# NVIDIA/DeepLearningExamples

Measured on AMD Instinct MI355X. Metric: training samples/sec, higher is better.
Workload: dtype bf16; 1 GPU; ResNet-50 v1.5 (PyTorch/Classification/ConvNets) synthetic ImageNet 224x224, label smoothing 0.1, SGD momentum 0.875 (BASELINE.json configs[1]); batch_per_gpu=256, global_batch=256, layout=NHWC, hip_graph=False, parallelism=single GPU

## Files before the change

### deeplearningexamples_amd/_cabi.py

```python
import ctypes
import os

import torch

_HERE = os.path.dirname(os.path.abspath(__file__))
LIB_PATH = os.environ.get("DLE_LIB_PATH") or os.path.join(_HERE, "lib", "libdle_mi355x.so")

F32, F16, BF16 = 0, 1, 2
ACT_NONE, ACT_RELU, ACT_GELU, ACT_RELU_BWD, ACT_ADD, ACT_GELU_BWD, ACT_TANH, ACT_TANH_BWD = 0, 1, 2, 3, 4, 5, 6, 7
ACT_ADD_MASKED, ACT_MUL, ACT_GELU_DAUX = 8, 9, 10

_DT = {torch.float32: F32, torch.float16: F16, torch.bfloat16: BF16}

c_void_p, c_int, c_i64, c_float = ctypes.c_void_p, ctypes.c_int, ctypes.c_int64, ctypes.c_float
c_u64 = ctypes.c_uint64

_SIGS = {
    "dle_last_error": (ctypes.c_char_p, []),
    "dle_abi_version": (c_int, []),
    "dle_device_check": (c_int, [c_int, ctypes.c_char_p, c_int]),
    "dle_dot_interact_out_width": (c_int, [c_int, c_int]),
    "dle_dot_interact_fwd": (c_int, [c_void_p, c_void_p, c_int, c_int, c_int, c_int, c_int, c_void_p]),
    "dle_dot_interact_bwd": (c_int, [c_void_p, c_void_p, c_void_p, c_void_p, c_int, c_int, c_int, c_int,
                                     c_int, c_void_p]),
# ... 17 lines not shown
    "dle_emb_sgd_workspace_bytes": (c_i64, [c_void_p, c_int, c_int, c_i64]),
    "dle_emb_onehot_try": (c_int, [c_void_p, c_void_p, c_void_p, c_void_p, c_float, c_void_p, c_void_p, c_void_p, c_void_p,
                                   c_void_p, c_int, c_i64, c_int, c_int, c_i64, c_int, c_void_p, c_i64, c_void_p]),
    "dle_emb_onehot_partials": (c_int, [c_void_p, c_void_p, c_void_p, c_void_p, c_void_p, c_void_p, c_int, c_i64, c_int, c_int,
                                        c_i64, c_int, c_void_p, c_i64, c_void_p, c_void_p]),
    "dle_emb_adam_workspace_bytes": (c_i64, [c_void_p, c_int, c_int, c_i64]),
    "dle_emb_adam_dedup_ws": (c_int, [c_void_p] * 9 + [c_float, c_void_p, c_void_p, c_void_p, c_float, c_float, c_float, c_i64,
                                      c_int, c_int, c_i64, c_int, c_void_p, c_i64, c_void_p]),
    "dle_cast_rows": (c_int, [c_void_p, c_void_p, c_i64, c_int, c_int, c_i64, c_i64, c_int, c_int, c_void_p]),
    "dle_bce_logits": (c_int, [c_void_p, c_void_p, c_void_p, c_void_p, c_void_p, c_i64, c_i64, c_int, c_void_p]),
    "dle_conv1x1_bnbwd_dgrad": (c_int, [c_void_p] * 16 + [c_i64, c_int, c_int, c_int, c_int, c_void_p]),
    "dle_conv1x1_bnbwd_groups": (c_int, [c_int]),
    "dle_conv1x1_bnbwd_dgrad_wgrad": (c_int, [c_void_p] * 15 + [c_i64, c_void_p, c_void_p, c_void_p, c_i64, c_int, c_int, c_int, c_int,
                                              c_void_p]),
    "dle_conv1x1_bnbwd_wgrad_workspace": (c_i64, [c_int, c_int]),
    "dle_gemm_expand_masked_bnred": (c_int, [c_void_p] * 10 + [c_i64, c_int, c_int, c_int, c_i64, c_i64, c_i64, c_int, c_int, c_void_p]),
    "dle_bn_bwd_finish": (c_int, [c_void_p, c_int, c_int, c_void_p, c_void_p, c_int, c_void_p]),
    "dle_gemm_colsum": (c_int, [c_void_p, c_void_p, c_void_p, c_void_p, c_void_p, c_int, c_int, c_int, c_i64, c_i64, c_i64, c_int,
                                c_int, c_int, c_void_p, c_i64, c_void_p]),
    "dle_head_bce_workspace_bytes": (c_i64, [c_i64, c_int]),
    "dle_head_bce_fwd_bwd": (c_int, [c_void_p, c_void_p, c_void_p, c_void_p, c_void_p, c_void_p, c_void_p, c_void_p, c_void_p,
                                     c_void_p, c_void_p, c_void_p, c_i64, c_i64, c_int, c_i64, c_i64, c_int, c_void_p]),
    "dle_amp_update_scale": (c_int, [c_void_p, c_void_p, c_void_p, c_void_p, c_float, c_float, c_int, c_int,
                                     c_void_p]),
    "dle_check_nonfinite": (c_int, [c_void_p, c_void_p, c_i64, c_int, c_void_p]),
    "dle_axpby_f32": (c_int, [c_void_p, c_void_p, c_void_p, c_float, c_float, c_i64, c_void_p]),
    "dle_act_bwd": (c_int, [c_void_p, c_void_p, c_void_p, c_i64, c_int, c_int, c_void_p]),
    "dle_relu_bwd": (c_int, [c_void_p, c_void_p, c_void_p, c_i64, c_int, c_i64, c_i64, c_i64, c_int, c_void_p]),
    "dle_gemm": (c_int, [c_void_p, c_void_p, c_void_p, c_void_p, c_void_p, c_void_p, c_int, c_int, c_int,
                         c_i64, c_i64, c_i64, c_int, c_int, c_int, c_int, c_int, c_int, c_int, c_float,
# ... 339 lines not shown
```

### deeplearningexamples_amd/convnets/resnet.py

```python
from contextlib import nullcontext as _nullcontext
from typing import List

import os

import torch
from torch import nn

from .. import _cabi as C
from .. import functional as F

LAYERS, WIDTHS, EXPANSION = [3, 4, 6, 3], [64, 128, 256, 512], 4


def _conv(cin, cout, k, stride, device):
    m = nn.Conv2d(cin, cout, kernel_size=k, stride=stride, padding=(k - 1) // 2, bias=False, device=device)
    nn.init.kaiming_normal_(m.weight, mode="fan_in", nonlinearity="relu")
    m.weight.data = m.weight.data.contiguous(memory_format=torch.channels_last)
    return m


def _bn(c, device, zero_init=False):
    m = nn.BatchNorm2d(c, device=device)
    nn.init.constant_(m.weight, 0 if zero_init else 1)
    nn.init.constant_(m.bias, 0)
# ... 29 lines not shown

class ConvBN:

    def __init__(self, conv: nn.Conv2d, bn: nn.BatchNorm2d, name_conv: str, name_bn: str, relu: bool):
        self.conv, self.bn, self.name_conv, self.name_bn, self.relu = conv, bn, name_conv, name_bn, relu
        self.k = conv.kernel_size[0]
        self.stride, self.pad = conv.stride[0], conv.padding[0]
        self.cin, self.cout = conv.in_channels, conv.out_channels
        self.w16 = None
        self.gw = self.ggamma = self.gbeta = None
        self.saved = None
        self.w2 = self.gw_flat = None
        self.wgrad_stream = None
        self.fuse_bnbwd = os.environ.get("DLE_RN50_FUSE_BNBWD", "1") != "0"
        self.fuse_bnbwd_wgrad = os.environ.get("DLE_RN50_FUSE_BNBWD_WGRAD", "1") != "0"
        self.reduce_done = False
        self.keepalive = None

    def forward(self, x, residual=None, defer=False):
        t = None
        if isinstance(x, Deferred):
            d, r = x, None
            if self.k == 1 and self.stride == 1 and d.unit.relu and d.y is None:
                res, res_bn = d.residual_args()
                r = F.conv1x1_bnload_fwd(d.t, res, self.w16, d.mean, d.rstd, d.unit.bn.weight.data, d.unit.bn.bias.data,
                                         self.bn.running_mean, self.bn.running_var, eps=self.bn.eps, momentum=self.bn.momentum,
                                         res_bn=res_bn)
            if r is not None:
                t, x, bits, mean, rstd = r
                d._done(x, bits)
# ... 35 lines not shown
        fused = None
        wgrad_done = False
        if self.fuse_bnbwd and self.k == 1 and self.stride == 1 and need_dx and dx_addend is None:
            b2 = None
            if bnred is not None and bnred.saved is not None and bnred.relu:
                b2 = (bnred.saved[1], bnred.saved[2], bnred.saved[3], bnred.saved[4], bnred.ggamma, bnred.gbeta)
            if self.fuse_bnbwd_wgrad and pooled is None and self.gw is not None:
                r = F.bn_bwd_conv1x1_dgrad_wgrad(dy, t, mean, rstd, self.bn.weight.data, self.ggamma, self.gbeta,
                                                 self.w16.view(self.cout, c), x, self.gw, relu_mask=rmask,
                                                 reduce_done=reduce_done, bnred=b2)
                if r is not None:
                    fused, wgrad_done = (None, r[0], r[1]), True
            if fused is None:
                fused = F.bn_bwd_conv1x1_dgrad(dy, t, mean, rstd, self.bn.weight.data, self.ggamma, self.gbeta,
                                               self.w16.view(self.cout, c), relu_mask=rmask, reduce_done=reduce_done, bnred=b2)
        gt = None
        if pooled is not None:
            if self.relu and not reduce_done:
                gt = F.pool_bn_bwd(pooled[0], pooled[1], t, mean, rstd, self.bn.weight.data, self.ggamma, self.gbeta, rmask)
            if gt is None:
                dy = F.maxpool_bwd(pooled[0], pooled[1], t.shape[1:3])
        if gt is not None:
            pass
        elif fused is not None:
            gt = fused[0]
            if fused[2]:
                bnred.reduce_done = True
        else:
            gt, _ = F.bn_bwd(dy, None, t, mean, rstd, self.bn.weight.data, self.ggamma, self.gbeta, relu_mask=rmask,
                             reduce_done=reduce_done)
# ... 110 lines not shown
```

### deeplearningexamples_amd/csrc/conv_bnbwd.hip

```cpp
#include "gemm_tiles.h"

#define BB_PAD 8

struct BnbArgs {
  const unsigned short* DY;
  const unsigned short* T;
  const unsigned char* bits;
  const unsigned short* B;
  unsigned short* DT;
  unsigned short* C;
  const float* mean; const float* rstd; const float* gamma; const float* dgamma; const float* dbeta;
  float inv_m;
  int M, N, K;
  int row_tiles, groups;
  const unsigned short* X;
  float* wpartial;
  float* tile_part;
  const unsigned short* t2;
  const unsigned char* bits2;
  const float* mean2; const float* rstd2;
  float* partial;
};

template <int DT> struct BbMfma;
// ... 51 lines not shown
  float* mu2 = cf + 5 * K;
  constexpr int WG_BASE = TN * LDW * 2 + 5 * K * 4 + 2 * TN * 4, LD = K * 2, LX = TN * 2;
  constexpr int KSL = K / NW, KB = KSL / 32, CB = TN / 32, MS = TM / 16, XP = TM * LX / 16 / (NW * 64);
  static_assert(!WG || (WG_BASE % 256 == 0 && KS == 8 && NB == 4 && XP * NW * 64 * 16 == TM * LX), "LDS image of the weight-gradient tile");
  unsigned char* dtl = smem_raw + WG_BASE;
  unsigned char* xl = dtl + TM * LD;
  const int lane = threadIdx.x & 63, wave = threadIdx.x >> 6;
  const int fr = lane & 15, kg = lane >> 4;
  const int g = blockIdx.x;
  for (int c = threadIdx.x; c < K * (TN / 8); c += NW * 64) {
    const int k = c / (TN / 8), nc = c - k * (TN / 8);
    const ushort8_t v = *(const ushort8_t*)(p.B + (long long)k * p.N + nc * 8);
#pragma unroll
    for (int e = 0; e < 8; ++e) wl[bb_pos(nc * 8 + e) * LDW + k] = v[e];
  }
  for (int c = threadIdx.x; c < K; c += NW * 64) {
    const float rs = p.rstd[c];
    cf[c] = p.gamma[c] * rs;
    cf[K + c] = p.mean[c];
    cf[2 * K + c] = rs;
    cf[3 * K + c] = p.dbeta[c] * p.inv_m;
    cf[4 * K + c] = p.dgamma[c] * p.inv_m;
  }
  if (BRED) {
    for (int c = threadIdx.x; c < TN; c += NW * 64) { mu2[c] = p.mean2[c]; mu2[TN + c] = p.rstd2[c]; }
  }
  __syncthreads();
  const unsigned short* wrow = wl + fr * LDW + kg * 8;
  const int mrow = wave * 16 + fr;
  ushort8_t fg[KS], fx[KS];
  uint4_t mb0, mb1;
  ushort8_t t2c[BRED ? NP : 1];
  uint2_t m2c;
  float r1 = 0.f, r2 = 0.f;
  ushort8_t xr[WG ? XP : 1];
  float16_t wacc[WG ? KB : 1][WG ? CB : 1];
  if constexpr (WG) {
#pragma unroll
// ... 30 lines not shown
#pragma unroll
      for (int i = 0; i < XP; ++i) {
        const int c = threadIdx.x + i * NW * 64, xm = tmn * TM + (c >> 3);
        xr[i] = *(const ushort8_t*)(p.X + (long long)(xm < p.M ? xm : p.M - 1) * TN + (c & 7) * 8);
      }
    }
  };
  load_rows(g);
  for (int tm = g; tm < p.row_tiles; tm += p.groups) {
    const int m_cur = tm * TM + mrow;
    const bool live = m_cur < p.M;
    {
      const long long o = (long long)(live ? m_cur : 0) * K + kg * 8;
#pragma unroll
      for (int ks = 0; ks < KS; ++ks) {
        const int c0 = ks * 32 + kg * 8;
        float gf[8], xf[8], of[8];
        unpack8<DT>(fg[ks], gf);
        unpack8<DT>(fx[ks], xf);
        const unsigned mw = ks < 4 ? mb0[ks & 3] : mb1[ks & 3];
        const unsigned bits = MASK ? (mw >> (8 * kg)) & 0xffu : 0xffu;
#pragma unroll
        for (int k = 0; k < 8; ++k) {
          if (MASK) { if (!((bits >> k) & 1u)) gf[k] = 0.f; }
          const float xh = (xf[k] - cf[K + c0 + k]) * cf[2 * K + c0 + k];
          of[k] = cf[c0 + k] * (gf[k] - cf[3 * K + c0 + k] - xh * cf[4 * K + c0 + k]);
        }
        fg[ks] = pack8<DT>(of);
        if constexpr (!WG) { if (live) *(ushort8_t*)(p.DT + o + ks * 32) = fg[ks]; }
      }
    }
    if constexpr (WG) {
      lds_barrier();
      const ushort8_t zero8 = {0, 0, 0, 0, 0, 0, 0, 0};
#pragma unroll
      for (int ks = 0; ks < KS; ++ks)
        *(ushort8_t*)(dtl + mrow * LD + (((ks * 2 + (kg >> 1)) ^ (2 * (mrow & 3))) << 5) + (kg & 1) * 16) = live ? fg[ks] : zero8;
#pragma unroll
      for (int i = 0; i < XP; ++i) {
        const int c = threadIdx.x + i * NW * 64, r = c >> 3, ch = c & 7;
        *(ushort8_t*)(xl + r * LX + (((ch >> 1) ^ (2 * ((r >> 1) & 1))) << 5) + (ch & 1) * 16) = tm * TM + r < p.M ? xr[i] : zero8;
      }
      lds_barrier();
// ... 240 lines not shown
```

### deeplearningexamples_amd/csrc/gemm_expand.hip

```cpp
#include "gemm_tiles.h"

#define EX_TN 128
#define EX_PAD 8

struct ExpandArgs {
  const unsigned short* A;
  const unsigned short* B;
  unsigned short* C;
  const unsigned short* src;
  const unsigned char* bits;
  float* stats;
  int M, N, K;
  long long lda, ldb, ldc;
  int b_kc, row_tiles, groups, col_tiles;
  FastDiv dHW, dW;
  int up_HW, up_W, up_P, up_Q;
  long long ld_src;
  const unsigned short* t2;
  const unsigned char* bits2;
  const float* mean2;
  const float* rstd2;
};

template <int DT> struct ExMfma;
template <> struct ExMfma<DLE_F16> {
  static __device__ __forceinline__ float4_t run(ushort8_t a, ushort8_t b, float4_t c) {
    return __builtin_amdgcn_mfma_f32_16x16x32_f16(__builtin_bit_cast(half8_t, a), __builtin_bit_cast(half8_t, b), c, 0, 0, 0);
  }
};
template <> struct ExMfma<DLE_BF16> {
  static __device__ __forceinline__ float4_t run(ushort8_t a, ushort8_t b, float4_t c) {
    return __builtin_amdgcn_mfma_f32_16x16x32_bf16(__builtin_bit_cast(bf16x8_t, a), __builtin_bit_cast(bf16x8_t, b), c, 0, 0, 0);
  }
};

__device__ __forceinline__ int ex_pos(int nl) {
  const int j = nl >> 5, r = nl & 31;
  return 32 * j + 16 * ((r >> 2) & 1) + 4 * (r >> 3) + (r & 3);
}

template <int KS, int ACT, bool BRED = false>
struct ExStream {
  ushort8_t fa[KS];
  ushort8_t sv[ACT ? 4 : 1];
  ushort8_t tv[BRED ? 4 : 1];
  uint4_t mb;
  uint4_t mb2;
  long long o0;
  bool live;
  bool has;
  __device__ __forceinline__ void load_a(const ExpandArgs& p, int m, int kg) {
    const long long mr = m < p.M ? m : p.M - 1;
    const unsigned short* arow = p.A + mr * p.lda + kg * 8;
#pragma unroll
    for (int ks = 0; ks < KS; ++ks) fa[ks] = *(const ushort8_t*)(arow + ks * 32);
  }
  __device__ __forceinline__ void load_src(const ExpandArgs& p, int m, int n0, int kg) {
    live = m < p.M;
    const long long mr = live ? m : p.M - 1;
    o0 = mr * p.ldc + n0 + kg * 8;
    if (ACT == 3) {
      const int mi = (int)mr;
      const int n = fd_div(mi, p.dHW), rem = mi - n * p.up_HW;
      const int h = fd_div(rem, p.dW), w = rem - h * p.up_W;
      has = !((h | w) & 1);
      const long long cr = has ? ((long long)n * p.up_P + (h >> 1)) * p.up_Q + (w >> 1) : 0;
      const unsigned short* srow = p.src + cr * p.ld_src + n0 + kg * 8;
#pragma unroll
      for (int j = 0; j < 4; ++j) sv[j] = *(const ushort8_t*)(srow + 32 * j);
    } else if (ACT) {
// ... 22 lines not shown
    const float keep = h4 ? w16[8 + q] : w16[q], send = h4 ? w16[q] : w16[8 + q];
    w8[q] = keep + __shfl_xor(send, 4, 64);
  }
#pragma unroll
  for (int q = 0; q < 4; ++q) {
    const float keep = h2 ? w8[4 + q] : w8[q], send = h2 ? w8[q] : w8[4 + q];
    w4[q] = keep + __shfl_xor(send, 2, 64);
  }
#pragma unroll
  for (int q = 0; q < 2; ++q) {
    const float keep = h1 ? w4[2 + q] : w4[q], send = h1 ? w4[q] : w4[2 + q];
    acc[q] += keep + __shfl_xor(send, 1, 64);
  }
}

template <int DT, int KS, int ACT, bool STATS, int NW, bool BRED = false>
__global__ __launch_bounds__(NW * 64) __attribute__((amdgpu_waves_per_eu((STATS || BRED) ? 3 : 4)))
void gemm_expand_kernel(ExpandArgs p) {
  constexpr int K = KS * 32, LDW = K + EX_PAD, TM = NW * 16;
  extern __shared__ __attribute__((aligned(16))) unsigned char smem_raw[];
  unsigned short* wl = (unsigned short*)smem_raw;
  const int lane = threadIdx.x & 63, wave = threadIdx.x >> 6;
  const int fr = lane & 15, kg = lane >> 4;
  const int xcd = blockIdx.x & 7, slot = blockIdx.x >> 3;
  const int tn = slot % p.col_tiles, g = (slot / p.col_tiles) * 8 + xcd;
  const int n0 = tn * EX_TN;
  if (p.b_kc) {
    constexpr int CPR = K / 8;
    for (int c = threadIdx.x; c < EX_TN * CPR; c += NW * 64) {
      const int nl = c / CPR, kc = c - nl * CPR;
      const ushort8_t v = *(const ushort8_t*)(p.B + (long long)(n0 + nl) * p.ldb + kc * 8);
      *(ushort8_t*)(wl + ex_pos(nl) * LDW + kc * 8) = v;
    }
  } else {
    for (int c = threadIdx.x; c < K * (EX_TN / 8); c += NW * 64) {
      const int k = c >> 4, nc = c & 15;
      const ushort8_t v = *(const ushort8_t*)(p.B + (long long)k * p.ldb + n0 + nc * 8);
#pragma unroll
      for (int e = 0; e < 8; ++e) wl[ex_pos(nc * 8 + e) * LDW + k] = v[e];
    }
  }
  float* mu2 = (float*)(smem_raw + EX_TN * LDW * 2);
  if (BRED) {
    for (int c = threadIdx.x; c < EX_TN; c += NW * 64) { mu2[c] = p.mean2[n0 + c]; mu2[EX_TN + c] = p.rstd2[n0 + c]; }
  }
  __syncthreads();
  float s1[STATS ? 32 : 1], s2[STATS ? 32 : 1];
  if (STATS) {
#pragma unroll
    for (int i = 0; i < 32; ++i) { s1[i] = 0.f; s2[i] = 0.f; }
  }
  float b1[2] = {0.f, 0.f}, b2s[2] = {0.f, 0.f};
  const unsigned short* wrow = wl + fr * LDW + kg * 8;
  const int mrow = wave * 16 + fr;
  ExStream<KS, ACT, BRED> cur;
  cur.load_a(p, g * TM + mrow, kg);
  cur.load_src(p, g * TM + mrow, n0, kg);
  for (int tm = g; tm < p.row_tiles; tm += p.groups) {
    const int m_next = (tm + p.groups) * TM + mrow;
    float4_t acc[8];
#pragma unroll
    for (int b = 0; b < 8; ++b) acc[b] = (float4_t){0.f, 0.f, 0.f, 0.f};
#pragma unroll
    for (int ks = 0; ks < KS; ++ks) {
#pragma unroll
      for (int b = 0; b < 8; ++b) {
        const ushort8_t fw = *(const ushort8_t*)(wrow + b * 16 * LDW + ks * 32);
        acc[b] = ExMfma<DT>::run(fw, cur.fa[ks], acc[b]);
      }
      __builtin_amdgcn_sched_barrier(0);
    }
    cur.load_a(p, m_next, kg);
    ushort8_t outv[4];
    float tg[BRED ? 32 : 1], tx[BRED ? 32 : 1];
    const bool live_cur = cur.live;
    const bool has_cur = ACT == 3 ? cur.has : true;
#pragma unroll
    for (int j = 0; j < 4; ++j) {
      float v[8];
#pragma unroll
      for (int r = 0; r < 4; ++r) { v[r] = acc[2 * j][r]; v[4 + r] = acc[2 * j + 1][r]; }
      if (ACT) {
        float y[8];
        unpack8<DT>(cur.sv[j], y);
        const unsigned int bits8 = ACT == 2 ? (cur.mb[j] >> (8 * kg)) & 0xffu : 0xffu;
#pragma unroll
        for (int r = 0; r < 8; ++r) {
// ... 45 lines not shown
      const long long o_other = odd ? o_own - p.ldc : o_own + p.ldc;
#pragma unroll
      for (int h = 0; h < 2; ++h) {
        const uint4_t mine0 = __builtin_bit_cast(uint4_t, outv[2 * h]), mine1 = __builtin_bit_cast(uint4_t, outv[2 * h + 1]);
        const uint4_t give = odd ? mine0 : mine1;
        uint4_t got;
#pragma unroll
        for (int q = 0; q < 4; ++q) got[q] = (unsigned)__shfl_xor((int)give[q], 1, 64);
        const uint4_t first = odd ? got : mine0, second = odd ? mine1 : got;
        const long long o_first = (odd ? o_other : o_own) + 64 * h + (odd ? 32 : 0);
        const long long o_second = (odd ? o_own : o_other) + 64 * h + (odd ? 32 : 0);
        const bool live_first = odd ? live_other : live_cur, live_second = odd ? live_cur : live_other;
        if (live_first) *(uint4_t*)(p.C + o_first) = first;
        if (live_second) *(uint4_t*)(p.C + o_second) = second;
      }
    }
  }
  if (BRED) {
    __syncthreads();
    float* red = (float*)smem_raw;
#pragma unroll
    for (int b = 0; b < 2; ++b) {
      const int i = 2 * fr + b, col = 32 * (i >> 3) + 8 * kg + (i & 7);
      red[(wave * 2 + 0) * EX_TN + col] = b1[b];
      red[(wave * 2 + 1) * EX_TN + col] = b2s[b];
    }
    __syncthreads();
    for (int t = threadIdx.x; t < 2 * EX_TN; t += NW * 64) {
      const int which = t / EX_TN, col = t - which * EX_TN;
      float tot = 0.f;
// ... 143 lines not shown
  const int lds_bytes = EX_TN * (K + EX_PAD) * 2;
  const dim3 grid((unsigned)(p.groups * p.col_tiles)), block(tmr * 4);
#define GO3(DT, KS)                                                                                                      \
  do {                                                                                                                   \
    constexpr int NW_ = KS > 4 ? 8 : 4;                                                                                  \
    DLE_LAUNCH_LDS((gemm_expand_kernel<DT, KS, 3, false, NW_>), grid, block, lds_bytes, stream, p);                      \
  } while (0)
#define PICK3(DT) do { if (K == 64) GO3(DT, 2); else if (K == 128) GO3(DT, 4); else GO3(DT, 8); } while (0)
  if (dtype == DLE_F16) PICK3(DLE_F16); else PICK3(DLE_BF16);
#undef PICK3
#undef GO3
  hipError_t e = hipGetLastError();
  if (e != hipSuccess) { dle_set_error("gemm_expand_add_up2 launch failed: %s", hipGetErrorString(e)); return (int)e + 1000; }
  return 1;
}
```

### deeplearningexamples_amd/csrc/gemm_tiles.h

```cpp
#pragma once
#include "gemm_family.h"
#include <type_traits>

struct FastDiv {
  unsigned mul, shr;
  int d;
};
static FastDiv make_fastdiv(int d) {
  FastDiv f;
  f.d = d;
  if (d <= 1) { f.mul = 0; f.shr = 0; return f; }
  unsigned lg = 0;
  while ((1u << lg) < (unsigned)d) ++lg;
  const unsigned p = 31 + lg;
  f.mul = (unsigned)(((1ull << p) + (unsigned)d - 1) / (unsigned)d);
  f.shr = p - 32;
  return f;
}
__device__ __forceinline__ int fd_div(int n, const FastDiv& f) {
  return f.d <= 1 ? n : (int)(__umulhi((unsigned)n, f.mul) >> f.shr);
}

struct ConvGeom {
  int H, W, C;
// ... 233 lines not shown
  if constexpr (ANY_RC) {
    asm volatile("s_waitcnt lgkmcnt(0)" ::: "memory");
    __builtin_amdgcn_sched_barrier(0);
  }
}

__device__ __forceinline__ void lds_barrier() { asm volatile("s_waitcnt lgkmcnt(0)\n\ts_barrier" ::: "memory"); }

template <int I, int N, class F>
__device__ __forceinline__ void static_for(F&& f) {
  if constexpr (I < N) {
    f(std::integral_constant<int, I>());
    static_for<I + 1, N>(f);
  }
}
```

### deeplearningexamples_amd/functional.py

```python
import ctypes
import os

import torch

from . import _cabi as C


def dot_interact_out_width(rows, cols):
    return C.lib().dle_dot_interact_out_width(rows, cols)


def dot_interact_fwd(x, force_generic=False):
    C.require_cuda(x)
    if x.dim() != 3:
        raise ValueError("dot_interact: expected [batch, rows, cols], got %s" % (tuple(x.shape),))
    x = x.contiguous()
    b, r, c = x.shape
    out = torch.empty((b, dot_interact_out_width(r, c)), dtype=x.dtype, device=x.device)
    C.annotate(bytes=float(b) * (r * c + out.shape[1]) * x.element_size())
    C.call("dle_dot_interact_fwd", C.ptr(x), C.ptr(out), b, r, c, C.dt(x), int(force_generic), C.stream())
    return out


def dot_interact_bwd(x, upstream, force_generic=False, fuse_mlp_grad=False, grad_out=None, found_inf=None):
# ... 1260 lines not shown
            gemm(dt.view(m, k), xin.view(m, n), k, n, m, False, False, out=gw.view(k, n),
                 splitk=pick_splitk(k, n, m, target_blocks=1024))
        return (None if wg else dt), dx, False
    if t2 is not None:
        C.call("dle_bn_bwd_finish", C.ptr(part), groups, n, C.ptr(bnred[4]), C.ptr(bnred[5]), 0, C.stream())
    return dt, dx, t2 is not None


def bn_bwd_conv1x1_dgrad(dy, x, mean, rstd, gamma, dgamma, dbeta, w, relu_mask=None, reduce_done=False, bnred=None):
    return _bn_bwd_conv1x1(dy, x, mean, rstd, gamma, dgamma, dbeta, w, relu_mask, reduce_done, bnred)


def bn_bwd_conv1x1_dgrad_wgrad(dy, x, mean, rstd, gamma, dgamma, dbeta, w, xin, gw, relu_mask=None, reduce_done=False, bnred=None):
    out = _bn_bwd_conv1x1(dy, x, mean, rstd, gamma, dgamma, dbeta, w, relu_mask, reduce_done, bnred, xin, gw)
    return out and out[1:]


def maxpool_fwd(x, ksize=3, stride=2, pad=1):
    C.require_cuda(x)
    n, h, w, c = x.shape
    p, q = (h + 2 * pad - ksize) // stride + 1, (w + 2 * pad - ksize) // stride + 1
    y = torch.empty((n, p, q, c), dtype=x.dtype, device=x.device)
    am = torch.empty((n, p, q, c), dtype=torch.uint8, device=x.device)
    C.annotate(bytes=float(x.numel() + y.numel()) * 2 + am.numel())
    C.call("dle_maxpool_fwd", C.ptr(x), C.ptr(y), C.ptr(am), n, h, w, c, ksize, stride, pad, C.dt(x), C.stream())
    return y, am


def maxpool_bwd(dy, argmax, in_hw, ksize=3, stride=2, pad=1):
    C.require_cuda(dy, argmax)
# ... 1026 lines not shown
```

### include/dle_mi355x.h

```cpp
#ifndef DLE_MI355X_H
#define DLE_MI355X_H
#include <stdint.h>

#ifdef __cplusplus
extern "C" {
#endif

typedef struct ihipStream_t* hipStream_t;

enum { DLE_F32 = 0, DLE_F16 = 1, DLE_BF16 = 2 };
enum { DLE_ACT_NONE = 0, DLE_ACT_RELU = 1, DLE_ACT_GELU = 2, DLE_ACT_RELU_BWD = 3, DLE_ACT_ADD = 4,
       DLE_ACT_GELU_BWD = 5, DLE_ACT_TANH = 6, DLE_ACT_TANH_BWD = 7,
       DLE_ACT_ADD_MASKED = 8,
       DLE_ACT_MUL = 9,
       DLE_ACT_GELU_DAUX = 10   };

const char* dle_last_error(void);
int dle_abi_version(void);
int dle_device_check(int device, char* arch_name, int arch_name_len);

int dle_dot_interact_out_width(int rows, int cols);
int dle_dot_interact_fwd(const void* x, void* out, int batch, int rows, int cols, int dtype,
                         int force_generic, hipStream_t stream);
int dle_dot_interact_bwd(const void* x, const void* upstream, void* grad, void* mlp_grad,
// ... 200 lines not shown
int dle_conv1x1_bnbwd_dgrad(const void* dy, const void* t, const void* relu_mask, const void* w, void* dt, void* dx,
                            const float* mean, const float* rstd, const float* gamma, const float* dgamma, const float* dbeta,
                            const void* t2, const void* bits2, const float* mean2, const float* rstd2, float* partial,
                            int64_t partial_bytes, int M, int N, int K, int dtype, hipStream_t stream);
int dle_conv1x1_bnbwd_groups(int M);
int dle_conv1x1_bnbwd_dgrad_wgrad(const void* dy, const void* t, const void* relu_mask, const void* w, void* dx,
                                  const float* mean, const float* rstd, const float* gamma, const float* dgamma,
                                  const float* dbeta, const void* t2, const void* bits2, const float* mean2, const float* rstd2,
                                  float* partial, int64_t partial_bytes, const void* x, float* gw, void* workspace,
                                  int64_t workspace_bytes, int M, int N, int K, int dtype, hipStream_t stream);
int64_t dle_conv1x1_bnbwd_wgrad_workspace(int M, int bnred);
int dle_gemm_expand_masked_bnred(const void* A, const void* B, void* C, const void* src, const void* bits, const void* t2,
                                 const void* bits2, const float* mean2, const float* rstd2, float* partial, int64_t partial_bytes,
                                 int M, int N, int K, int64_t lda, int64_t ldb, int64_t ldc, int b_kc, int dtype, hipStream_t stream);
int dle_bn_bwd_finish(const float* partial, int groups, int C, float* dgamma, float* dbeta, int accumulate, hipStream_t stream);
int dle_stem_conv7_groups(int N, int H);
int dle_stem_conv7_fwd(const void* x4, const void* w2, void* y, float* stats, int64_t stats_bytes, int N, int H, int W,
                       int dtype, hipStream_t stream);
int64_t dle_stem_conv7_wgrad_workspace(int N, int H);
int dle_stem_conv7_wgrad(const void* dy, const void* x4, float* dw, void* workspace, int64_t workspace_bytes, int N, int H,
                         int W, int dtype, int accumulate, hipStream_t stream);
int dle_stem_pack_weight(const float* w_krsc, void* out, int dtype, hipStream_t stream);
int dle_maxpool_fwd(const void* x, void* y, void* argmax, int N, int H, int W, int C, int ksize, int stride,
                    int pad, int dtype, hipStream_t stream);
int dle_bn_relu_maxpool_fwd(const void* x, void* y, void* argmax, void* relu_mask, const float* mean, const float* rstd,
                            const float* gamma, const float* beta, int N, int H, int W, int C, int dtype, hipStream_t stream);
int dle_maxpool_bwd(const void* dy, const void* argmax, void* dx, int N, int H, int W, int C, int ksize,
                    int stride, int pad, int dtype, hipStream_t stream);
int64_t dle_pool_bn_bwd_workspace_bytes(int N, int H, int W, int C);
int dle_pool_bn_bwd(const void* dy, const void* argmax, const void* relu_mask, const void* x, void* dz, const float* mean,
// ... 253 lines not shown
```

Before: 13410 samples/s.

## Fuse BN backward, expand dgrad and weight gradient for first bottleneck 1x1 conv

Adds a fused kernel for the first 1x1 conv in the bottleneck (K=64 or 128, N=256) in backward. It applies the BN backward transform to the incoming gradient on the fly, runs the expand-style dgrad GEMM with the residual addend (and the optional next BN reduction), and in the same pass accumulates the weight gradient via LDS transposed reads and MFMA into per-group partials that are later folded. This removes separate BN-backward and wgrad kernels and their extra activation reads and writes. In exchange the kernel uses more LDS and registers (waves_per_eu 2), needs a larger workspace, and adds a fold pass. The BN elementwise math is also refactored into shared helpers.

```diff
diff --git a/deeplearningexamples_amd/_cabi.py b/deeplearningexamples_amd/_cabi.py
--- a/deeplearningexamples_amd/_cabi.py
+++ b/deeplearningexamples_amd/_cabi.py
@@ -55,6 +55,9 @@
     "dle_conv1x1_bnbwd_dgrad_wgrad": (c_int, [c_void_p] * 15 + [c_i64, c_void_p, c_void_p, c_void_p, c_i64, c_int, c_int, c_int, c_int,
                                               c_void_p]),
     "dle_conv1x1_bnbwd_wgrad_workspace": (c_i64, [c_int, c_int]),
+    "dle_conv1x1_expand_bnbwd_dgrad_wgrad": (c_int, [c_void_p] * 12 + [c_int, c_int] + [c_void_p] * 5 + [c_i64, c_void_p, c_void_p,
+                                                     c_void_p, c_i64, c_int, c_int, c_int, c_int, c_void_p]),
+    "dle_conv1x1_expand_bnbwd_workspace": (c_i64, [c_int, c_int, c_int]),
     "dle_gemm_expand_masked_bnred": (c_int, [c_void_p] * 10 + [c_i64, c_int, c_int, c_int, c_i64, c_i64, c_i64, c_int, c_int, c_void_p]),
     "dle_bn_bwd_finish": (c_int, [c_void_p, c_int, c_int, c_void_p, c_void_p, c_int, c_void_p]),
     "dle_gemm_colsum": (c_int, [c_void_p, c_void_p, c_void_p, c_void_p, c_void_p, c_int, c_int, c_int, c_i64, c_i64, c_i64, c_int,
diff --git a/deeplearningexamples_amd/convnets/resnet.py b/deeplearningexamples_amd/convnets/resnet.py
--- a/deeplearningexamples_amd/convnets/resnet.py
+++ b/deeplearningexamples_amd/convnets/resnet.py
@@ -67,6 +67,7 @@
         self.wgrad_stream = None
         self.fuse_bnbwd = os.environ.get("DLE_RN50_FUSE_BNBWD", "1") != "0"
         self.fuse_bnbwd_wgrad = os.environ.get("DLE_RN50_FUSE_BNBWD_WGRAD", "1") != "0"
+        self.fuse_bn1bwd_wgrad = os.environ.get("DLE_RN50_FUSE_BN1BWD_WGRAD", "1") != "0"
         self.reduce_done = False
         self.keepalive = None
 
@@ -132,6 +133,20 @@
             if fused is None:
                 fused = F.bn_bwd_conv1x1_dgrad(dy, t, mean, rstd, self.bn.weight.data, self.ggamma, self.gbeta,
                                                self.w16.view(self.cout, c), relu_mask=rmask, reduce_done=reduce_done, bnred=b2)
+        if (self.fuse_bn1bwd_wgrad and self.k == 1 and self.stride == 1 and self.relu and need_dx and pooled is None
+                and isinstance(dx_addend, tuple) and self.gw is not None):
+            b3 = None
+            if dx_addend[0] != "up2" and bnred is not None and bnred.saved is not None and bnred.relu:
+                b3 = (bnred.saved[1], bnred.saved[2], bnred.saved[3], bnred.saved[4], bnred.ggamma, bnred.gbeta)
+            r = F.bn_bwd_conv1x1_expand_dgrad_wgrad(dy, t, mean, rstd, self.bn.weight.data, self.ggamma, self.gbeta,
+                                                    self.w16.view(self.cout, c), x, self.gw, rmask, dx_addend,
+                                                    reduce_done=reduce_done, bnred=b3)
+            if r is False:
+                reduce_done = True
+            elif r is not None:
+                if b3 is not None:
+                    bnred.reduce_done = True
+                return r.view(n, h, w, c)
         gt = None
         if pooled is not None:
             if self.relu and not reduce_done:
diff --git a/deeplearningexamples_amd/csrc/conv_bnbwd.hip b/deeplearningexamples_amd/csrc/conv_bnbwd.hip
--- a/deeplearningexamples_amd/csrc/conv_bnbwd.hip
+++ b/deeplearningexamples_amd/csrc/conv_bnbwd.hip
@@ -89,14 +89,7 @@
 #pragma unroll
     for (int e = 0; e < 8; ++e) wl[bb_pos(nc * 8 + e) * LDW + k] = v[e];
   }
-  for (int c = threadIdx.x; c < K; c += NW * 64) {
-    const float rs = p.rstd[c];
-    cf[c] = p.gamma[c] * rs;
-    cf[K + c] = p.mean[c];
-    cf[2 * K + c] = rs;
-    cf[3 * K + c] = p.dbeta[c] * p.inv_m;
-    cf[4 * K + c] = p.dgamma[c] * p.inv_m;
-  }
+  bn_bwd_coeffs(cf, K, p.mean, p.rstd, p.gamma, p.dgamma, p.dbeta, p.inv_m, threadIdx.x, NW * 64);
   if (BRED) {
     for (int c = threadIdx.x; c < TN; c += NW * 64) { mu2[c] = p.mean2[c]; mu2[TN + c] = p.rstd2[c]; }
   }
@@ -157,19 +150,9 @@
       const long long o = (long long)(live ? m_cur : 0) * K + kg * 8;
 #pragma unroll
       for (int ks = 0; ks < KS; ++ks) {
-        const int c0 = ks * 32 + kg * 8;
-        float gf[8], xf[8], of[8];
-        unpack8<DT>(fg[ks], gf);
-        unpack8<DT>(fx[ks], xf);
         const unsigned mw = ks < 4 ? mb0[ks & 3] : mb1[ks & 3];
         const unsigned bits = MASK ? (mw >> (8 * kg)) & 0xffu : 0xffu;
-#pragma unroll
-        for (int k = 0; k < 8; ++k) {
-          if (MASK) { if (!((bits >> k) & 1u)) gf[k] = 0.f; }
-          const float xh = (xf[k] - cf[K + c0 + k]) * cf[2 * K + c0 + k];
-          of[k] = cf[c0 + k] * (gf[k] - cf[3 * K + c0 + k] - xh * cf[4 * K + c0 + k]);
-        }
-        fg[ks] = pack8<DT>(of);
+        fg[ks] = bn_bwd_frag8<DT, MASK>(fg[ks], fx[ks], bits, cf, K, ks * 32 + kg * 8);
         if constexpr (!WG) { if (live) *(ushort8_t*)(p.DT + o + ks * 32) = fg[ks]; }
       }
     }
diff --git a/deeplearningexamples_amd/csrc/gemm_expand.hip b/deeplearningexamples_amd/csrc/gemm_expand.hip
--- a/deeplearningexamples_amd/csrc/gemm_expand.hip
+++ b/deeplearningexamples_amd/csrc/gemm_expand.hip
@@ -20,6 +20,12 @@
   const unsigned char* bits2;
   const float* mean2;
   const float* rstd2;
+  const unsigned short* t1;
+  const unsigned char* bits1;
+  const float* mean1; const float* rstd1; const float* gamma1; const float* dgamma1; const float* dbeta1;
+  float inv_m;
+  const unsigned short* X;
+  float* wpartial;
 };
 
 template <int DT> struct ExMfma;
@@ -39,8 +45,13 @@
   return 32 * j + 16 * ((r >> 2) & 1) + 4 * (r >> 3) + (r & 3);
 }
 
-template <int KS, int ACT, bool BRED = false>
-struct ExStream {
+template <int KS, bool BNW> struct ExStreamBnw {};
+template <int KS> struct ExStreamBnw<KS, true> {
+  ushort8_t ft[KS];
+  uint4_t mk;
+};
+template <int KS, int ACT, bool BRED = false, bool BNW = false>
+struct ExStream : ExStreamBnw<KS, BNW> {
   ushort8_t fa[KS];
   ushort8_t sv[ACT ? 4 : 1];
   ushort8_t tv[BRED ? 4 : 1];
@@ -54,6 +65,18 @@
     const unsigned short* arow = p.A + mr * p.lda + kg * 8;
 #pragma unroll
     for (int ks = 0; ks < KS; ++ks) fa[ks] = *(const ushort8_t*)(arow + ks * 32);
+    if constexpr (BNW) {
+      static_assert(KS == 2 || KS == 4, "the row's keep bytes are one 8- or 16-byte load");
+      const unsigned short* trow = p.t1 + mr * (KS * 32) + kg * 8;
+#pragma unroll
+      for (int ks = 0; ks < KS; ++ks) this->ft[ks] = *(const ushort8_t*)(trow + ks * 32);
+      if (KS == 2) {
+        const uint2_t m2 = *(const uint2_t*)(p.bits1 + mr * (KS * 4));
+        this->mk[0] = m2[0]; this->mk[1] = m2[1];
+      } else {
+        this->mk = *(const uint4_t*)(p.bits1 + mr * (KS * 4));
+      }
+    }
   }
   __device__ __forceinline__ void load_src(const ExpandArgs& p, int m, int n0, int kg) {
     live = m < p.M;
@@ -106,12 +129,28 @@
   }
 }
 
-template <int DT, int KS, int ACT, bool STATS, int NW, bool BRED = false>
-__global__ __launch_bounds__(NW * 64) __attribute__((amdgpu_waves_per_eu((STATS || BRED) ? 3 : 4)))
+template <int OFF>
+__device__ __forceinline__ short4_t ex_tr(unsigned addr) {
+  short4_t v;
+  asm volatile("ds_read_b64_tr_b16 %0, %1 offset:%2" : "=v"(v) : "v"(addr), "n"(OFF) : "memory");
+  return v;
+}
+
+constexpr int ex_bnw_base(int K, bool bred) { return (EX_TN * (K + EX_PAD) * 2 + (bred ? 2 * EX_TN * 4 : 0) + 5 * K * 4 + 255) / 256 * 256; }
+template <int L> __device__ __forceinline__ int ex_swz(int r) { return L == 128 ? ((r >> 1) & 1) : (r & 3); }
+
+template <int DT, int KS, int ACT, bool STATS, int NW, bool BRED = false, bool BNW = false>
+__global__ __launch_bounds__(NW * 64) __attribute__((amdgpu_waves_per_eu(BNW ? 2 : (STATS || BRED) ? 3 : 4)))
 void gemm_expand_kernel(ExpandArgs p) {
   constexpr int K = KS * 32, LDW = K + EX_PAD, TM = NW * 16;
   extern __shared__ __attribute__((aligned(16))) unsigned char smem_raw[];
   unsigned short* wl = (unsigned short*)smem_raw;
+  constexpr int WG_BASE = ex_bnw_base(K, BRED), LD = K * 2, LX = EX_TN * 2;
+  constexpr int WM = KS / 2, WN = 2, MS = TM / 16, XP = TM * LX / 16 / (NW * 64);
+  static_assert(!BNW || (NW == 4 && !STATS && XP * NW * 64 * 16 == TM * LX), "BNW: 4 wavefronts as 2 x 2 over [K][128]");
+  float* cf = (float*)(smem_raw + WG_BASE - 5 * K * 4);
+  unsigned char* dtl = smem_raw + WG_BASE;
+  unsigned char* xl = dtl + TM * LD;
   const int lane = threadIdx.x & 63, wave = threadIdx.x >> 6;
   const int fr = lane & 15, kg = lane >> 4;
   const int xcd = blockIdx.x & 7, slot = blockIdx.x >> 3;
@@ -136,7 +175,32 @@
   if (BRED) {
     for (int c = threadIdx.x; c < EX_TN; c += NW * 64) { mu2[c] = p.mean2[n0 + c]; mu2[EX_TN + c] = p.rstd2[n0 + c]; }
   }
+  if constexpr (BNW) bn_bwd_coeffs(cf, K, p.mean1, p.rstd1, p.gamma1, p.dgamma1, p.dbeta1, p.inv_m, threadIdx.x, NW * 64);
   __syncthreads();
+  float16_t wacc[BNW ? WM : 1][BNW ? WN : 1];
+  ushort8_t xr[BNW ? XP : 1];
+  const int wm = wave >> 1, wn = wave & 1;
+  const int tr_row = (kg >> 1) * 8 + (fr >> 2);
+  const unsigned lds0 = (unsigned)(unsigned long)(__attribute__((address_space(3))) unsigned char*)smem_raw;
+  const unsigned da0 = lds0 + WG_BASE + tr_row * LD + (kg & 1) * 32 + (fr & 3) * 8;
+  const unsigned xa0 = lds0 + WG_BASE + TM * LD + tr_row * LX + (kg & 1) * 32 + (fr & 3) * 8;
+  if constexpr (BNW) {
+#pragma unroll
+    for (int i = 0; i < WM; ++i)
+#pragma unroll
+      for (int j = 0; j < WN; ++j)
+#pragma unroll
+        for (int r = 0; r < 16; ++r) wacc[i][j][r] = 0.f;
+  }
+  auto load_x = [&](int tile) __attribute__((always_inline)) {
+    if constexpr (BNW) {
+#pragma unroll
+      for (int i = 0; i < XP; ++i) {
+        const int c = threadIdx.x + i * NW * 64, xm = tile * TM + (c >> 4);
+        xr[i] = *(const ushort8_t*)(p.X + (long long)(xm < p.M ? xm : p.M - 1) * p.N + n0 + (c & 15) * 8);
+      }
+    }
+  };
   float s1[STATS ? 32 : 1], s2[STATS ? 32 : 1];
   if (STATS) {
 #pragma unroll
@@ -145,11 +209,52 @@
   float b1[2] = {0.f, 0.f}, b2s[2] = {0.f, 0.f};
   const unsigned short* wrow = wl + fr * LDW + kg * 8;
   const int mrow = wave * 16 + fr;
-  ExStream<KS, ACT, BRED> cur;
+  ExStream<KS, ACT, BRED, BNW> cur;
   cur.load_a(p, g * TM + mrow, kg);
+  load_x(g);
   cur.load_src(p, g * TM + mrow, n0, kg);
   for (int tm = g; tm < p.row_tiles; tm += p.groups) {
     const int m_next = (tm + p.groups) * TM + mrow;
+    if constexpr (BNW) {
+#pragma unroll
+      for (int ks = 0; ks < KS; ++ks)
+        cur.fa[ks] = bn_bwd_frag8<DT, true>(cur.fa[ks], cur.ft[ks], (cur.mk[ks] >> (8 * kg)) & 0xffu, cf, K, ks * 32 + kg * 8);
+      lds_barrier();
+      const ushort8_t zero8 = {0, 0, 0, 0, 0, 0, 0, 0};
+      const bool live_row = tm * TM + mrow < p.M;
+#pragma unroll
+      for (int ks = 0; ks < KS; ++ks)
+        *(ushort8_t*)(dtl + mrow * LD + ((ks ^ ex_swz<LD>(mrow)) << 6) + kg * 16) = live_row ? cur.fa[ks] : zero8;
+#pragma unroll
+      for (int i = 0; i < XP; ++i) {
+        const int c = threadIdx.x + i * NW * 64, r = c >> 4, ch = c & 15;
+        *(ushort8_t*)(xl + r * LX + (((ch >> 2) ^ ex_swz<LX>(r)) << 6) + (ch & 3) * 16) = tm * TM + r < p.M ? xr[i] : zero8;
+      }
+      lds_barrier();
+      static_for<0, MS>([&](auto S) __attribute__((always_inline)) {
+        constexpr int s = decltype(S)::value;
+        TrPair ta[WM], tb[WN];
+#pragma unroll
+        for (int i = 0; i < WM; ++i) {
+          const unsigned a = da0 + (((wm * WM + i) ^ ex_swz<LD>(tr_row)) << 6);
+          ta[i].lo = ex_tr<s * 16 * LD>(a);
+          ta[i].hi = ex_tr<(s * 16 + 4) * LD>(a);
+        }
+#pragma unroll
+        for (int j = 0; j < WN; ++j) {
+          const unsigned a = xa0 + (((wn * WN + j) ^ ex_swz<LX>(tr_row)) << 6);
+          tb[j].lo = ex_tr<s * 16 * LX>(a);
+          tb[j].hi = ex_tr<(s * 16 + 4) * LX>(a);
+        }
+        frag_wait<true>();
+#pragma unroll
+        for (int i = 0; i < WM; ++i) {
+          const ushort8_t va = frag_value(ta[i]);
+#pragma unroll
+          for (int j = 0; j < WN; ++j) wacc[i][j] = Mfma32x16<DT>::run(va, frag_value(tb[j]), wacc[i][j]);
+        }
+      });
+    }
     float4_t acc[8];
 #pragma unroll
     for (int b = 0; b < 8; ++b) acc[b] = (float4_t){0.f, 0.f, 0.f, 0.f};
@@ -163,6 +268,7 @@
       __builtin_amdgcn_sched_barrier(0);
     }
     cur.load_a(p, m_next, kg);
+    load_x(tm + p.groups);
     ushort8_t outv[4];
     float tg[BRED ? 32 : 1], tx[BRED ? 32 : 1];
     const bool live_cur = cur.live;
@@ -238,6 +344,18 @@
         if (live_first) *(uint4_t*)(p.C + o_first) = first;
         if (live_second) *(uint4_t*)(p.C + o_second) = second;
       }
+    }
+  }
+  if constexpr (BNW) {
+    if (g < p.row_tiles) {
+      float* out = p.wpartial + (long long)g * (K * p.N) + n0;
+#pragma unroll
+      for (int i = 0; i < WM; ++i)
+#pragma unroll
+        for (int j = 0; j < WN; ++j)
+#pragma unroll
+          for (int r = 0; r < 16; ++r)
+            out[(long long)((wm * WM + i) * 32 + 8 * (r >> 2) + 4 * (lane >> 5) + (r & 3)) * p.N + (wn * WN + j) * 32 + (lane & 31)] = wacc[i][j][r];
     }
   }
   if (BRED) {
@@ -411,3 +529,67 @@
   if (e != hipSuccess) { dle_set_error("gemm_expand_add_up2 launch failed: %s", hipGetErrorString(e)); return (int)e + 1000; }
   return 1;
 }
+
+static int ex_bnw_cap(int K) { return K == 64 ? 512 : 256; }
+static int ex_bnw_groups(int M, int K) {
+  const int row_tiles = (M + 63) / 64, cap = ex_bnw_cap(K);
+  return ((row_tiles < cap ? row_tiles : cap) + 7) / 8 * 8;
+}
+extern "C" int64_t dle_conv1x1_expand_bnbwd_workspace(int M, int N, int K) {
+  if (M < 8192 || N != 256 || (K != 64 && K != 128)) return 0;
+  const int row_tiles = (M + 63) / 64, cap = ex_bnw_cap(K);
+  return (int64_t)(row_tiles < cap ? row_tiles : cap) * K * N * 4;
+}
+
+extern "C" int dle_conv1x1_expand_bnbwd_dgrad_wgrad(const void* dy1, const void* t1, const void* bits1, const void* w, void* dx,
+                                                    const float* mean1, const float* rstd1, const float* gamma1,
+                                                    const float* dgamma1, const float* dbeta1, const void* src,
+                                                    const void* src_bits, int H, int W, const void* t2, const void* bits2,
+                                                    const float* mean2, const float* rstd2, float* partial, int64_t partial_bytes,
+                                                    const void* x, float* gw, void* workspace, int64_t workspace_bytes, int M,
+                                                    int N, int K, int dtype, hipStream_t stream) {
+  if (!dle_gemm_expand_enabled()) return 0;
+  if (dtype != DLE_F16 && dtype != DLE_BF16) return 0;
+  const int64_t need = dle_conv1x1_expand_bnbwd_workspace(M, N, K);
+  if (need == 0 || workspace_bytes < need) return 0;
+  const int only = dle_env_int("DLE_EXPAND_BNBWD_K", 0);
+  if (only && only != K) return 0;
+  if (!dy1 || !t1 || !bits1 || !w || !dx || !mean1 || !rstd1 || !gamma1 || !dgamma1 || !dbeta1 || !src || !x || !gw || !workspace) return 0;
+  const bool up2 = K == 128;
+  if (up2) {
+    if (src_bits || t2 || (H & 1) || (W & 1) || H <= 0 || W <= 0 || (M % (H * W)) != 0) return 0;
+  } else {
+    if (!src_bits || !t2 || !bits2 || !mean2 || !rstd2 || !partial) return 0;
+  }
+  if (((((uintptr_t)dy1) | ((uintptr_t)t1) | ((uintptr_t)bits1) | ((uintptr_t)w) | ((uintptr_t)dx) | ((uintptr_t)src) |
+        ((uintptr_t)src_bits) | ((uintptr_t)t2) | ((uintptr_t)bits2) | ((uintptr_t)x) | ((uintptr_t)gw) | ((uintptr_t)workspace)) & 15) != 0)
+    return 0;
+  ExpandArgs p = {(const unsigned short*)dy1, (const unsigned short*)w, (unsigned short*)dx, (const unsigned short*)src,
+                  (const unsigned char*)src_bits, partial, M, N, K, (long long)K, (long long)N, (long long)N, 0, 0, 0, 0};
+  p.t2 = (const unsigned short*)t2; p.bits2 = (const unsigned char*)bits2; p.mean2 = mean2; p.rstd2 = rstd2;
+  p.t1 = (const unsigned short*)t1; p.bits1 = (const unsigned char*)bits1;
+  p.mean1 = mean1; p.rstd1 = rstd1; p.gamma1 = gamma1; p.dgamma1 = dgamma1; p.dbeta1 = dbeta1; p.inv_m = 1.0f / (float)M;
+  p.X = (const unsigned short*)x; p.wpartial = (float*)workspace;
+  if (up2) {
+    p.dHW = make_fastdiv(H * W); p.dW = make_fastdiv(W);
+    p.up_HW = H * W; p.up_W = W; p.up_P = H / 2; p.up_Q = W / 2; p.ld_src = N;
+  }
+  p.row_tiles = (M + 63) / 64;
+  p.col_tiles = N / EX_TN;
+  p.groups = ex_bnw_groups(M, K);
+  if (!up2 && (p.groups != dle_gemm_expand_groups(M, N, K) || partial_bytes < (long long)p.groups * 2 * N * 4)) return 0;
+  const size_t lds_bytes = (size_t)ex_bnw_base(K, !up2) + (size_t)64 * (K + EX_TN) * 2;
+  const dim3 grid((unsigned)(p.groups * p.col_tiles)), block(256);
+  if (up2) {
+    if (dtype == DLE_F16) DLE_LAUNCH_LDS((gemm_expand_kernel<DLE_F16, 4, 3, false, 4, false, true>), grid, block, lds_bytes, stream, p);
+    else DLE_LAUNCH_LDS((gemm_expand_kernel<DLE_BF16, 4, 3, false, 4, false, true>), grid, block, lds_bytes, stream, p);
+  } else {
+    if (dtype == DLE_F16) DLE_LAUNCH_LDS((gemm_expand_kernel<DLE_F16, 2, 2, false, 4, true, true>), grid, block, lds_bytes, stream, p);
+    else DLE_LAUNCH_LDS((gemm_expand_kernel<DLE_BF16, 2, 2, false, 4, true, true>), grid, block, lds_bytes, stream, p);
+  }
+  hipError_t e = hipGetLastError();
+  if (e != hipSuccess) { dle_set_error("conv1x1_expand_bnbwd_dgrad_wgrad launch failed: %s", hipGetErrorString(e)); return (int)e + 1000; }
+  e = wgrad1x1_fold((const float*)workspace, gw, (long long)K * N / 4, (int)(need / ((int64_t)K * N * 4)), 0, stream);
+  if (e != hipSuccess) { dle_set_error("conv1x1_expand_bnbwd_dgrad_wgrad fold launch failed: %s", hipGetErrorString(e)); return (int)e + 1000; }
+  return 1;
+}
diff --git a/deeplearningexamples_amd/csrc/gemm_tiles.h b/deeplearningexamples_amd/csrc/gemm_tiles.h
--- a/deeplearningexamples_amd/csrc/gemm_tiles.h
+++ b/deeplearningexamples_amd/csrc/gemm_tiles.h
@@ -271,3 +271,28 @@
     static_for<I + 1, N>(f);
   }
 }
+
+__device__ __forceinline__ void bn_bwd_coeffs(float* cf, int K, const float* mean, const float* rstd, const float* gamma,
+                                              const float* dgamma, const float* dbeta, float inv_m, int tid, int nthreads) {
+  for (int c = tid; c < K; c += nthreads) {
+    const float rs = rstd[c];
+    cf[c] = gamma[c] * rs;
+    cf[K + c] = mean[c];
+    cf[2 * K + c] = rs;
+    cf[3 * K + c] = dbeta[c] * inv_m;
+    cf[4 * K + c] = dgamma[c] * inv_m;
+  }
+}
+template <int DT, bool MASK>
+__device__ __forceinline__ ushort8_t bn_bwd_frag8(ushort8_t g16, ushort8_t t16, unsigned bits, const float* cf, int K, int c0) {
+  float gf[8], xf[8], of[8];
+  unpack8<DT>(g16, gf);
+  unpack8<DT>(t16, xf);
+#pragma unroll
+  for (int k = 0; k < 8; ++k) {
+    if (MASK) { if (!((bits >> k) & 1u)) gf[k] = 0.f; }
+    const float xh = (xf[k] - cf[K + c0 + k]) * cf[2 * K + c0 + k];
+    of[k] = cf[c0 + k] * (gf[k] - cf[3 * K + c0 + k] - xh * cf[4 * K + c0 + k]);
+  }
+  return pack8<DT>(of);
+}
diff --git a/deeplearningexamples_amd/functional.py b/deeplearningexamples_amd/functional.py
--- a/deeplearningexamples_amd/functional.py
+++ b/deeplearningexamples_amd/functional.py
@@ -1298,6 +1298,69 @@
 def bn_bwd_conv1x1_dgrad_wgrad(dy, x, mean, rstd, gamma, dgamma, dbeta, w, xin, gw, relu_mask=None, reduce_done=False, bnred=None):
     out = _bn_bwd_conv1x1(dy, x, mean, rstd, gamma, dgamma, dbeta, w, relu_mask, reduce_done, bnred, xin, gw)
     return out and out[1:]
+
+
+def bn_bwd_conv1x1_expand_dgrad_wgrad(dy, x, mean, rstd, gamma, dgamma, dbeta, w, xin, gw, relu_mask, addend, reduce_done=False,
+                                      bnred=None):
+    k = x.shape[-1]
+    m = x.numel() // k
+    n = w.shape[-1]
+    up2 = isinstance(addend, tuple) and len(addend) == 3 and addend[0] == "up2"
+    if not up2 and not (isinstance(addend, tuple) and len(addend) == 2 and bnred is not None):
+        return None
+    src = addend[1] if up2 else addend[0]
+    more = (src,) if up2 else (src, addend[1]) + tuple(bnred)
+    C.require_cuda(dy, x, mean, rstd, gamma, dgamma, dbeta, w, xin, gw, relu_mask, *more)
+    if (relu_mask is None or x.dtype not in (torch.float16, torch.bfloat16) or w.numel() != k * n or k != (128 if up2 else 64)
+            or any(t.dtype != x.dtype for t in (dy, w, xin, src)) or gw.dtype != torch.float32 or gw.numel() != k * n
+            or xin.numel() != m * n or dy.numel() != m * k or not all(t.is_contiguous() for t in (dy, x, w, xin, src, gw))
+            or any(t.data_ptr() % 16 for t in (dy, x, w, xin, src, gw, relu_mask))
+            or os.environ.get("DLE_GEMM_EXPAND", "1") == "0"):
+        return None
+    h = wd = 0
+    t2 = bits2 = mean2 = rstd2 = src_bits = None
+    if up2:
+        h, wd = addend[2]
+        if h <= 0 or wd <= 0 or h % 2 or wd % 2 or m % (h * wd) or src.numel() * 4 != m * n:
+            return None
+    else:
+        src_bits = addend[1]
+        t2, bits2, mean2, rstd2 = bnred[:4]
+        if (src.numel() != m * n or t2.numel() != m * n or not t2.is_contiguous() or t2.dtype != x.dtype or bits2 is None
+                or any(t.data_ptr() % 16 for t in (src_bits, t2, bits2)) or os.environ.get("DLE_RN50_FUSE_BNRED", "1") == "0"):
+            return None
+    wg_bytes = int(C.lib().dle_conv1x1_expand_bnbwd_workspace(m, n, k))
+    if wg_bytes == 0:
+        return None
+    act_bytes = 0.125
+    if not reduce_done:
+        ws = _bn_ws(x.reshape(m, k))
+        C.annotate(bytes=float(x.numel()) * (4 + act_bytes), tag="M%dxC%d+relu" % (m, k))
+        C.call("dle_bn_bwd_reduce", C.ptr(dy), None, C.ptr(relu_mask), C.ptr(x), C.ptr(mean), C.ptr(rstd), C.ptr(dgamma),
+               C.ptr(dbeta), m, k, 0, C.ptr(ws), ws.numel() * 4, C.dt(x), C.stream())
+    groups = 0 if up2 else int(C.lib().dle_gemm_expand_groups(m, n, k))
+    part_bytes = (groups * 2 * n * 4 + 15) // 16 * 16
+    buf = splitk_workspace(x.device, part_bytes + wg_bytes)
+    part = None if up2 else buf[:part_bytes // 4]
+    wpart = buf[part_bytes // 4:]
+    dx = torch.empty((m, n), dtype=x.dtype, device=x.device)
+    es = x.element_size()
+    by = float(m) * k * (2 * es + act_bytes) + float(m) * n * 2 * es + float(k) * n * (es + 4) + float(wg_bytes) * 2
+    by += float(src.numel()) * es + (0.0 if up2 else float(m) * n * (es + 0.25))
+    C.annotate(bytes=by, flops=4.0 * m * n * k, tag="bn_bwd+dgrad+wgrad %dx%dx%d%s" % (m, n, k, "+up2" if up2 else "+src+aux+bnred"))
+    name = "dle_conv1x1_expand_bnbwd_dgrad_wgrad"
+    rc = _timed_optional(name, getattr(C.lib(), name),
+                         (C.ptr(dy), C.ptr(x), C.ptr(relu_mask), C.ptr(w), C.ptr(dx), C.ptr(mean), C.ptr(rstd), C.ptr(gamma),
+                          C.ptr(dgamma), C.ptr(dbeta), C.ptr(src), C.ptr(src_bits), h, wd, C.ptr(t2), C.ptr(bits2), C.ptr(mean2),
+                          C.ptr(rstd2), C.ptr(part), part_bytes, C.ptr(xin), C.ptr(gw), C.ptr(wpart), wpart.numel() * 4, m, n, k,
+                          C.dt(x), C.stream()))
+    if rc > 1:
+        C.check(rc - 1000 if rc > 1000 else -1, name)
+    if rc != 1:
+        return None if reduce_done else False
+    if not up2:
+        C.call("dle_bn_bwd_finish", C.ptr(part), groups, n, C.ptr(bnred[4]), C.ptr(bnred[5]), 0, C.stream())
+    return dx
 
 
 def maxpool_fwd(x, ksize=3, stride=2, pad=1):
diff --git a/include/dle_mi355x.h b/include/dle_mi355x.h
--- a/include/dle_mi355x.h
+++ b/include/dle_mi355x.h
@@ -238,6 +238,13 @@
                                  const void* bits2, const float* mean2, const float* rstd2, float* partial, int64_t partial_bytes,
                                  int M, int N, int K, int64_t lda, int64_t ldb, int64_t ldc, int b_kc, int dtype, hipStream_t stream);
 int dle_bn_bwd_finish(const float* partial, int groups, int C, float* dgamma, float* dbeta, int accumulate, hipStream_t stream);
+int dle_conv1x1_expand_bnbwd_dgrad_wgrad(const void* dy1, const void* t1, const void* bits1, const void* w, void* dx,
+                                         const float* mean1, const float* rstd1, const float* gamma1, const float* dgamma1,
+                                         const float* dbeta1, const void* src, const void* src_bits, int H, int W, const void* t2,
+                                         const void* bits2, const float* mean2, const float* rstd2, float* partial,
+                                         int64_t partial_bytes, const void* x, float* gw, void* workspace, int64_t workspace_bytes,
+                                         int M, int N, int K, int dtype, hipStream_t stream);
+int64_t dle_conv1x1_expand_bnbwd_workspace(int M, int N, int K);
 int dle_stem_conv7_groups(int N, int H);
 int dle_stem_conv7_fwd(const void* x4, const void* w2, void* y, float* stats, int64_t stats_bytes, int N, int H, int W,
                        int dtype, hipStream_t stream);
```

Result: no change. 13490 samples/s, median of 6 (+0.6%).
